# foriequal0/homework-18-graphics-raytracer

Measured on AMD Instinct MI355X. Metric: Mrays/s (primary+secondary) at 1920x1080, depth 8, higher is better.
Workload: dtype f32

## Files before the change

### homework-18-graphics-raytracer_amd/csrc/rt_pwf.hip

```cpp
#include "rt_pwf_kernel.h"

namespace rt {

static size_t pwf_dynamic_lds(uint32_t node_cap, uint32_t ring_cap) {
    const bool packed = pa_ready_packed(node_cap, ring_cap);
    return (size_t)(PA_READY_WORDS((node_cap + 63u) / 64u, packed) + 2u * PA_READY_WORDS(ring_cap / 64u, packed)) * sizeof(uint32_t);
}

int pwf_workgroups_per_cu(uint32_t node_cap, uint32_t ring_cap, bool bfs_walk) {
    int n = 0;
    const size_t lds = pwf_dynamic_lds(node_cap, ring_cap);
    const bool packed = pa_ready_packed(node_cap, ring_cap);
    const hipError_t e = bfs_walk ? (packed ? hipOccupancyMaxActiveBlocksPerMultiprocessor(&n, pwf_kernel<true, true>, (int)PA_THREADS, lds)
                                            : hipOccupancyMaxActiveBlocksPerMultiprocessor(&n, pwf_kernel<false, true>, (int)PA_THREADS, lds))
                                  : (packed ? hipOccupancyMaxActiveBlocksPerMultiprocessor(&n, pwf_kernel<true, false>, (int)PA_THREADS, lds)
                                            : hipOccupancyMaxActiveBlocksPerMultiprocessor(&n, pwf_kernel<false, false>, (int)PA_THREADS, lds));
    if (e != hipSuccess || n < 1) n = 1;
    return n;
}

__global__ void pwf_init_kernel(uint32_t *global, KernelFrame *frame, const KernelFrame fr) {
    if (threadIdx.x < PW_G_BLOCK_WORDS) global[threadIdx.x] = 0u;
    if (threadIdx.x == 0u) *frame = fr;
}

size_t pwf_arena_bytes(uint32_t node_cap, uint32_t ring_cap, uint32_t max_depth) {
    return ((size_t)node_cap * 4u + (size_t)ring_cap * (3u + PA_SHADE_U4)) * sizeof(uint4) + (size_t)(node_cap / 64u) * 2u * sizeof(uint32_t) +
           (((size_t)node_cap + 15u) & ~(size_t)15u) + (size_t)pwf_fold_list_regions(max_depth) * node_cap * sizeof(uint32_t) + 256u;
}

#ifdef PA_STATS
static uint32_t *g_pw_last_global = nullptr;
extern "C" int rt_diag_read_pwf(uint32_t *out32) {
    if (!g_pw_last_global) return -1;
    return hipMemcpy(out32, g_pw_last_global, 32 * sizeof(uint32_t), hipMemcpyDeviceToHost) == hipSuccess ? 0 : -1;
}
extern "C" int rt_diag_read_pwf_phases(unsigned long long *out32, int reset) {
    if (hipMemcpyFromSymbol(out32, HIP_SYMBOL(pa_phase_stats), 32 * sizeof(unsigned long long)) != hipSuccess) return -1;
    if (reset) {
        unsigned long long zero[32] = {0};
        if (hipMemcpyToSymbol(HIP_SYMBOL(pa_phase_stats), zero, sizeof zero) != hipSuccess) return -1;
    }
    return 0;
}
#endif

hipError_t launch_pwf(const KernelScene &sc, KernelFrame fr, float *out, const PwParams &pp, uint32_t workgroups, hipStream_t stream,
                      bool init, bool first_band, bool last_band) {
    const uint32_t total = fr.cols * fr.rows;
    fr.n_chunks = (total + 63u) / 64u;
    if (total == 0u) return hipSuccess;
#ifdef PA_STATS
    g_pw_last_global = pp.global;
#endif
    if (init) hipLaunchKernelGGL(pwf_init_kernel, dim3(1), dim3(64), 0, stream, pp.global, const_cast<KernelFrame *>(pp.frame), fr);
    if (first_band) record_main_kernel_event(0, stream);
    const size_t lds = pwf_dynamic_lds(pp.node_cap, pp.ring_cap);
    const bool packed = pa_ready_packed(pp.node_cap, pp.ring_cap);
    if (frame_is_rays(fr)) launch_pwf_rays(sc, pp, out, workgroups, lds, stream, packed, sc.bfs_walk != 0u && pp.bfs_scratch != nullptr);
    else launch_pwf_kernel<false>(sc, pp, out, workgroups, lds, stream, packed, sc.bfs_walk != 0u && pp.bfs_scratch != nullptr);
    if (last_band) record_main_kernel_event(1, stream);
    return hipGetLastError();
}

}

#ifdef RT_DIAG_STAGES
RT_DIAG_STAGE_READER(rt_diag_read_stages_pwf)
#endif
#ifdef RT_DIAG_NEED
RT_DIAG_NEED_READER(rt_diag_read_need_pwf)
#endif
#ifdef RT_DIAG_BFS
RT_DIAG_BFS_READER(rt_diag_read_bfs)
#endif
```

### homework-18-graphics-raytracer_amd/csrc/rt_pwf_kernel.h

```cpp
#ifndef RT_PWF_KERNEL_H
#define RT_PWF_KERNEL_H

#include <hip/hip_runtime.h>
#include <stdint.h>

#include "../../include/rt_amd.h"
#include "rt_device_scene.h"
#include "rt_shade.h"
#include "rt_kernels.h"
#include "rt_cast.h"
#include "rt_pwf_common.h"

namespace rt {

#ifndef PA_WAVES
#define PA_WAVES 8u
#endif
#define PA_THREADS (PA_WAVES * 64u)
#ifndef PA_MIN_WAVES
#define PA_MIN_WAVES 6
#endif
#ifndef PA_SHADE_PAGES
#define PA_SHADE_PAGES 4u
#endif
#ifndef PA_MIN_PARTIAL
#define PA_MIN_PARTIAL 1u
#endif
#ifndef PA_CHAIN_PARTIAL_MIN
#define PA_CHAIN_PARTIAL_MIN 1u
#endif
#ifndef PA_PRIO_CHAIN
#define PA_PRIO_CHAIN 1
#define PA_PRIO_TILE 1
#endif
#ifndef PA_SLEEP
#define PA_SLEEP 16
#endif
#define PA_SHADE_U4 5u
#ifndef PA_LDS_PAGES
#define PA_LDS_PAGES 2u
#endif
#ifndef PA_LQ
#define PA_LQ 3u
#endif
#define PA_LQ_SHIFT 4u
#ifndef PA_LDS_F_PAGES
#define PA_LDS_F_PAGES 2u
#endif
#ifndef PA_LDS_N_PAGES
#define PA_LDS_N_PAGES 2u
#endif
#ifndef PA_DRAIN_ROOM
#define PA_DRAIN_ROOM 64u
#endif
#define PA_IN_LDS 8u
#define PA_SPIN_LIMIT (1u << 22)

enum : uint32_t { PA_T_NONE = 0u, PA_T_NODE = 1u, PA_T_REFR = 2u, PA_T_TILE = 3u, PA_T_SHADE = 4u };

struct PaShared {
    PaQueue n, f, s;
    PaQueue l[PA_LQ];
    uint32_t l_released[PA_LQ];
    uint32_t ready_l[PA_LQ][PA_LDS_PAGES];
    PaQueue lf;
    uint32_t lf_released;
    uint32_t ready_lf[PA_LDS_F_PAGES];
    PaQueue ln;
    uint32_t ln_released;
    uint32_t ready_ln[PA_LDS_N_PAGES];
    uint32_t root_alloc;
    uint32_t tiles_exhausted;
    uint32_t tile_list_count;
    uint32_t static_next;
    uint32_t idle;
    uint32_t gen;
    uint32_t done;
    uint32_t abort;
    uint32_t fold_count[64];
};

template <class P>
__device__ __forceinline__ void pa_store_shade(P *t, uint32_t id, uint32_t prim, uint32_t word, V3 spos, V3 adj_n, V3 in_dir, V3 sdiffuse, V3 sum) {
    t[PA_F(0u)] = make_uint4(id, prim, word, 0u);
    t[PA_F(1u)] = make_uint4(pfu(spos.x), pfu(spos.y), pfu(spos.z), pfu(sum.x));
    t[PA_F(2u)] = make_uint4(pfu(adj_n.x), pfu(adj_n.y), pfu(adj_n.z), pfu(sum.y));
    t[PA_F(3u)] = make_uint4(pfu(in_dir.x), pfu(in_dir.y), pfu(in_dir.z), pfu(sum.z));
    t[PA_F(4u)] = make_uint4(pfu(sdiffuse.x), pfu(sdiffuse.y), pfu(sdiffuse.z), 0u);
}

template <class P>
__device__ __forceinline__ void pa_store_node(P *t, V3 o, V3 d, uint32_t word, float contribution, uint32_t id) {
    t[PA_F(0u)] = make_uint4(pfu(o.x), pfu(o.y), pfu(o.z), pfu(d.x));
    t[PA_F(1u)] = make_uint4(pfu(d.y), pfu(d.z), word, pfu(contribution));
    if (id != 0xffffffffu) t[PA_F(2u)] = make_uint4(id, 0u, 0u, 0u);
}

__device__ __forceinline__ uint32_t pa_top_node(uint32_t *root_alloc, const uint32_t *n_alloc, uint32_t node_cap, bool want, bool *overflow) {
    const unsigned long long mask = __builtin_amdgcn_ballot_w64(want);
    *overflow = false;
    if (mask == 0ull) return 0u;
    const uint32_t n = (uint32_t)__builtin_popcountll(mask);
    const int leader = (int)__builtin_ctzll(mask);
    uint32_t base = 0u;
    if ((int)(threadIdx.x & 63u) == leader) base = atomicAdd(root_alloc, n);
    base = (uint32_t)__builtin_amdgcn_readlane((int)base, leader);
    if (base + n + lds_load(n_alloc) > node_cap) { *overflow = want; return 0u; }
    return node_cap - 1u - (base + __builtin_amdgcn_mbcnt_hi((uint32_t)(mask >> 32), __builtin_amdgcn_mbcnt_lo((uint32_t)mask, 0u)));
}

template <class P>
__device__ __forceinline__ void pa_store_refr(P *t, V3 o, V3 d, uint32_t word, uint32_t parent, uint32_t obj, float contribution, float travel, uint32_t retry) {
    t[PA_F(0u)] = make_uint4(pfu(o.x), pfu(o.y), pfu(o.z), pfu(d.x));
    t[PA_F(1u)] = make_uint4(pfu(d.y), pfu(d.z), word, parent);
    t[PA_F(2u)] = make_uint4(obj, pfu(contribution), pfu(travel), retry);
}

__device__ __forceinline__ void pa_release_page(uint32_t *released, uint32_t page, uint32_t lane) {
    asm volatile("s_waitcnt lgkmcnt(0)" ::: "memory");
    if (lane == 0u) {
        while (lds_load(released) != page) __builtin_amdgcn_s_sleep(1);
        __hip_atomic_store(released, page + 1u, __ATOMIC_RELEASE, __HIP_MEMORY_SCOPE_WORKGROUP);
    }
}

#ifdef PA_STATS
__device__ unsigned long long pa_phase_stats[32];
#define PA_TICK() __builtin_readcyclecounter()
#endif

template <bool PACKED, bool BFS = false, bool RAYS = false>
__global__ __launch_bounds__(PA_THREADS, BFS ? 2 : PA_MIN_WAVES) void pwf_kernel(const KernelScene sc, const PwParams pp, float *__restrict__ out) {
    BfsLds *bfs_lds = nullptr;
    BfsScratch bfs_ws = {nullptr, nullptr, nullptr, 0u, 0u};
    if constexpr (BFS) {
        __shared__ BfsLds bfs_lds_all[PA_WAVES];
        bfs_lds = &bfs_lds_all[threadIdx.x >> 6];
        uint2 *const mine = reinterpret_cast<uint2 *>(pp.bfs_scratch) + ((size_t)blockIdx.x * PA_WAVES + (threadIdx.x >> 6)) * (2u * (size_t)pp.bfs_items_cap + pp.bfs_jobs_cap);
        bfs_ws.items_a = mine;
        bfs_ws.items_b = mine + pp.bfs_items_cap;
        bfs_ws.jobs = mine + 2u * (size_t)pp.bfs_items_cap;
        bfs_ws.items_cap = pp.bfs_items_cap;
        bfs_ws.jobs_cap = pp.bfs_jobs_cap;
    }
    extern __shared__ uint32_t pa_ready[];
    __shared__ PaShared S;
    __shared__ uint4 lds_shade[PA_LQ * PA_LDS_PAGES * PA_SHADE_U4 * 64u];
    __shared__ uint4 lds_refr[PA_LDS_F_PAGES * 3u * 64u];
    __shared__ uint4 lds_node[PA_LDS_N_PAGES * 3u * 64u];
    const auto &fr = uniform_ref(pp.frame);
    const uint32_t lane = threadIdx.x & 63u;
    const uint32_t total_slots = fr.cols * fr.rows;
    const uint32_t n_tiles = fr.n_chunks;
    const float THRESHOLD = 0.001f;

    unsigned char *arena = pp.arena + (size_t)blockIdx.x * pp.arena_stride;
    uint4 *node_in = reinterpret_cast<uint4 *>(arena);
    uint4 *nodes = node_in + (size_t)pp.node_cap * 2u;
    uint4 *shade_q = nodes + (size_t)pp.node_cap * 2u;
    uint4 *refr_q = shade_q + (size_t)pp.ring_cap * PA_SHADE_U4;
    uint32_t *tile_list = reinterpret_cast<uint32_t *>(refr_q + (size_t)pp.ring_cap * 3u);
    const uint32_t ring_mask = pp.ring_cap - 1u;
    const uint32_t tile_cap = pp.node_cap / 64u;
    unsigned char *root_mark = reinterpret_cast<unsigned char *>(((uintptr_t)(tile_list + (size_t)tile_cap * 2u) + 15u) & ~(uintptr_t)15u);
    uint32_t *fold_list = reinterpret_cast<uint32_t *>(root_mark + (((size_t)pp.node_cap + 15u) & ~(size_t)15u));
    auto fold_slot = [&](uint32_t level, uint32_t i) -> uint32_t * {
        uint32_t *region = fold_list + (size_t)((level - 1u) >> 1) * pp.node_cap;
        return region + (((level - 1u) & 1u) != 0u ? pp.node_cap - 1u - i : i);
    };
    const uint32_t node_pages = (pp.node_cap + 63u) / 64u, ring_pages = pp.ring_cap / 64u;
    uint32_t *ready_n = pa_ready, *ready_s = pa_ready + PA_READY_WORDS(node_pages, PACKED), *ready_f = ready_s + PA_READY_WORDS(ring_pages, PACKED);
    const uint32_t ring_page_mask = ring_pages - 1u;

    for (uint32_t i = threadIdx.x; i < PA_READY_WORDS(node_pages, PACKED) + 2u * PA_READY_WORDS(ring_pages, PACKED); i += PA_THREADS) pa_ready[i] = 0u;
    if (threadIdx.x < 64u) S.fold_count[threadIdx.x] = 0u;
    if (threadIdx.x == 0u) {
        S.n.alloc = S.n.taken = 0u;
        S.f.alloc = S.f.taken = 0u;
        S.s.alloc = S.s.taken = 0u;
        for (uint32_t q = 0; q < PA_LQ; ++q) {
            S.l[q].alloc = S.l[q].taken = 0u;
            S.l_released[q] = 0u;
            for (uint32_t k = 0; k < PA_LDS_PAGES; ++k) S.ready_l[q][k] = 0u;
        }
        S.lf.alloc = S.lf.taken = 0u;
        S.lf_released = 0u;
        for (uint32_t k = 0; k < PA_LDS_F_PAGES; ++k) S.ready_lf[k] = 0u;
        S.ln.alloc = S.ln.taken = 0u;
        S.ln_released = 0u;
        for (uint32_t k = 0; k < PA_LDS_N_PAGES; ++k) S.ready_ln[k] = 0u;
        S.root_alloc = 0u;
        S.tiles_exhausted = 0u;
        S.tile_list_count = 0u;
        S.static_next = 0u;
        S.idle = 0u;
        S.gen = 0u;
        S.done = 0u;
        S.abort = 0u;
    }
    __syncthreads();
    uint32_t casts = 0u;
    auto queue_shade = [&](bool want, uint32_t id, uint32_t prim, uint32_t word, uint32_t light_i, V3 spos, V3 adj_n, V3 in_dir, V3 sdiffuse, V3 sum) {
        const uint32_t mine = light_i < PA_LQ - 1u ? light_i : PA_LQ - 1u;
#pragma unroll
        for (uint32_t q = 0; q < PA_LQ; ++q) {
            const bool w = want && mine == q;
            if (__builtin_amdgcn_ballot_w64(w) == 0ull) continue;
            bool fits;
            const uint32_t k = pa_try_append_some(&S.l[q], &S.l_released[q], PA_LDS_PAGES * 64u, w, &fits);
            if (fits) pa_store_shade(lds_shade + q * (PA_LDS_PAGES * PA_SHADE_U4 * 64u) + pa_entry(k & (PA_LDS_PAGES * 64u - 1u), PA_SHADE_U4), id, prim, word, spos, adj_n, in_dir, sdiffuse, sum);
            pa_publish(S.ready_l[q], PA_LDS_PAGES - 1u, fits, k, &S.gen);
            want = want && !fits;
        }
#ifdef PA_STATS
        for (uint32_t q = 0; q < 3u; ++q) {
            const unsigned long long m = __builtin_amdgcn_ballot_w64(want && (mine < 2u ? mine : 2u) == q);
            if (m != 0ull && lane == (uint32_t)__builtin_ctzll(m)) atomicAdd(pp.global + 28 + q, (uint32_t)__builtin_popcountll(m));
        }
#endif
        const uint32_t k = lds_append(&S.s.alloc, want);
        if (want) pa_store_shade(shade_q + pa_entry(k & ring_mask, PA_SHADE_U4), id, prim, word, spos, adj_n, in_dir, sdiffuse, sum);
        pa_publish<PACKED>(ready_s, ring_page_mask, want, k, &S.gen);
    };
#ifdef PA_STATS
    const unsigned long long st_t0 = __builtin_amdgcn_s_memrealtime();
    uint32_t st_hist[5] = {0u, 0u, 0u, 0u, 0u};
    uint32_t st_shadow[3] = {0u, 0u, 0u};
    unsigned long long ph[26];
    for (int k = 0; k < 26; ++k) ph[k] = 0ull;
#endif

    for (;;) {
        if (lds_load(&S.done) != 0u || lds_load(&S.abort) != 0u) break;

#ifdef PA_STATS
        const unsigned long long ph_t0 = PA_TICK();
#endif
        uint32_t type = PA_T_NONE, start = 0u, count = 0u;
        if (lane == 0u) {
            const uint32_t gen = lds_load(&S.gen);
            auto look = [&]() -> uint32_t {
                const uint32_t a0 = lds_load(&S.ln.alloc), a1 = lds_load(&S.n.alloc), a2 = lds_load(&S.lf.alloc), a3 = lds_load(&S.f.alloc);
                const uint32_t t0 = lds_load(&S.ln.taken), t1 = lds_load(&S.n.taken), t2 = lds_load(&S.lf.taken), t3 = lds_load(&S.f.taken);
                uint32_t al[PA_LQ], tl[PA_LQ];
                for (uint32_t q = 0; q < PA_LQ; ++q) { al[q] = lds_load(&S.l[q].alloc); tl[q] = lds_load(&S.l[q].taken); }
                const uint32_t as = lds_load(&S.s.alloc), ts = lds_load(&S.s.taken);
                uint32_t m = (a0 > t0 * 64u ? 1u : 0u) | (a1 > t1 * 64u ? 2u : 0u) | (a2 > t2 * 64u ? 4u : 0u) | (a3 > t3 * 64u ? 8u : 0u);
                for (uint32_t q = 0; q < PA_LQ; ++q) m |= al[q] > tl[q] * 64u ? 16u << q : 0u;
                m |= as > ts * 64u ? 16u << PA_LQ : 0u;
                return m;
            };
            uint32_t have = look();
            auto claim_chain = [&](uint32_t min_partial) {
                if ((have & 1u) != 0u) {
                    count = pa_claim(&S.ln, S.ready_ln, PA_LDS_N_PAGES - 1u, min_partial, &start);
                    if (count != 0u) { type = PA_T_NODE | PA_IN_LDS; return; }
                }
                if ((have & 2u) != 0u) {
                    count = pa_claim<PACKED>(&S.n, ready_n, 0xffffffffu, min_partial, &start);
                    if (count != 0u) { type = PA_T_NODE; return; }
                }
                if ((have & 4u) != 0u) {
                    count = pa_claim(&S.lf, S.ready_lf, PA_LDS_F_PAGES - 1u, min_partial, &start);
                    if (count != 0u) { type = PA_T_REFR | PA_IN_LDS; return; }
                }
                if ((have & 8u) != 0u) {
                    count = pa_claim<PACKED>(&S.f, ready_f, ring_page_mask, min_partial, &start);
                    if (count != 0u) type = PA_T_REFR;
                }
            };
            auto claim_shade = [&](uint32_t min_partial) {
                for (uint32_t q = 0; q < PA_LQ; ++q) {
                    if ((have & (16u << q)) == 0u) continue;
                    count = pa_claim(&S.l[q], S.ready_l[q], PA_LDS_PAGES - 1u, min_partial, &start);
                    if (count != 0u) { type = PA_T_SHADE | PA_IN_LDS | (q << PA_LQ_SHIFT); return; }
                }
                if ((have & (16u << PA_LQ)) == 0u) return;
                count = pa_claim<PACKED>(&S.s, ready_s, ring_page_mask, min_partial, &start);
                if (count != 0u) type = PA_T_SHADE;
            };
            claim_chain(0u);
            if (PA_DRAIN_ROOM != 0u && type == PA_T_NONE && lds_load(&S.tiles_exhausted) == 0u) {
                for (uint32_t q = 0; q < PA_LQ; ++q) {
                    if (lds_load(&S.l[q].alloc) - (lds_load(&S.l_released[q]) << 6) + PA_DRAIN_ROOM > PA_LDS_PAGES * 64u) {
                        count = pa_claim(&S.l[q], S.ready_l[q], PA_LDS_PAGES - 1u, 0u, &start);
                        if (count != 0u) { type = PA_T_SHADE | PA_IN_LDS | (q << PA_LQ_SHIFT); break; }
                    }
                }
            }
            if (PA_CHAIN_PARTIAL_MIN != 0u && type == PA_T_NONE) claim_chain(PA_CHAIN_PARTIAL_MIN);
            bool tried_tile = false;
            for (int pass = 0; pass < 2 && type == PA_T_NONE; ++pass) {
                if (!tried_tile && lds_load(&S.tiles_exhausted) == 0u) {
                    uint32_t shade_pages = (lds_load(&S.s.alloc) >> 6) - lds_load(&S.s.taken);
                    for (uint32_t q = 0; q < PA_LQ; ++q) shade_pages += (lds_load(&S.l[q].alloc) >> 6) - lds_load(&S.l[q].taken);
                    if (pass == 1 || (int32_t)shade_pages < (int32_t)PA_SHADE_PAGES) {
                        tried_tile = true;
                        const uint32_t used = lds_load(&S.n.alloc) + lds_load(&S.root_alloc);
                        const uint32_t room = pp.node_cap > used ? pp.node_cap - used : 0u;
                        if (room < 64u * pp.tile_reserve || lds_load(&S.tile_list_count) >= tile_cap) {
                            S.tiles_exhausted = 1u;
                        } else {
                            const uint32_t share = n_tiles / gridDim.x;
                            const uint32_t own = share / 2u > (share < 8u ? share : 8u) ? share / 2u : (share < 8u ? share : 8u);
                            uint32_t k;
                            const uint32_t mine = own != 0u && lds_load(&S.static_next) < own ? atomicAdd(&S.static_next, 1u) : own;
                            if (mine < own) k = blockIdx.x + gridDim.x * mine;
                            else k = gridDim.x * own + atomicAdd(pp.global + PW_G_TILE, 1u);
                            if (k >= n_tiles) {
                                S.tiles_exhausted = 1u;
                            } else {
                                start = pp.tile_order != nullptr ? pp.tile_order[k] : (uint32_t)(((unsigned long long)k * pp.tile_stride) % n_tiles);
                                count = total_slots - start * 64u < 64u ? total_slots - start * 64u : 64u;
                                type = PA_T_TILE;
                            }
                        }
                    }
                }
                if (type == PA_T_NONE && pass == 0) claim_shade(0u);
            }
            for (int last = 0; last < 2 && type == PA_T_NONE; ++last) {
                const uint32_t min_partial = last ? 1u : PA_MIN_PARTIAL;
                have = look();
                claim_chain(min_partial);
                if (type != PA_T_NONE) break;
                claim_shade(min_partial);
                if (type != PA_T_NONE) break;
                if (last) {
                    if (lds_load(&S.idle) == PA_WAVES - 1u) S.done = 1u;
                    break;
                }
                if (atomicAdd(&S.idle, 1u) + 1u == PA_WAVES) {
                    atomicSub(&S.idle, 1u);
                    continue;
                }
                uint32_t spins = 0u;
                while (lds_load(&S.gen) == gen && lds_load(&S.done) == 0u && lds_load(&S.abort) == 0u) {
                    __builtin_amdgcn_s_sleep(PA_SLEEP);
                    if (++spins > PA_SPIN_LIMIT) {
                        S.abort = 1u;
                        atomicExch(pp.global + PW_G_OVERFLOW, 1u);
                    }
                }
                atomicSub(&S.idle, 1u);
                break;
            }
        }
        type = (uint32_t)__builtin_amdgcn_readfirstlane((int)type);
        start = (uint32_t)__builtin_amdgcn_readfirstlane((int)start);
        count = (uint32_t)__builtin_amdgcn_readfirstlane((int)count);
        const bool in_lds = (type & PA_IN_LDS) != 0u;
        const uint32_t lq = (type >> PA_LQ_SHIFT) & 3u;
        type &= 7u;
        const bool one_light = type == PA_T_SHADE && in_lds && (lq < PA_LQ - 1u || sc.n_lights <= PA_LQ);
#ifdef PA_STATS
        const unsigned long long ph_t1 = PA_TICK();
        if (type == PA_T_NONE) ph[24] += ph_t1 - ph_t0;
        const uint32_t ph_k = type == PA_T_NODE ? 0u : (type == PA_T_REFR ? 1u : (type == PA_T_TILE ? 2u : 3u));
#endif
        if (type == PA_T_NONE) continue;
        __builtin_amdgcn_fence(__ATOMIC_ACQUIRE, "workgroup");
        if (type == PA_T_SHADE) __builtin_amdgcn_s_setprio(0);
        else if (type == PA_T_TILE) __builtin_amdgcn_s_setprio(PA_PRIO_TILE);
        else __builtin_amdgcn_s_setprio(PA_PRIO_CHAIN);
#ifdef PA_STATS
        st_hist[count <= 8u ? 0 : (count <= 16u ? 1 : (count <= 32u ? 2 : (count < 64u ? 3 : 4)))] += 1u;
#endif

        const bool active = lane < count;
        Ray req;
        req.o = v3(0.0f, 0.0f, 0.0f);
        req.d = v3(0.0f, 0.0f, 1.0f);
        req.mode = FACE_FRONT;
        req.excl = 0u;
        bool do_cast = active;
        uint32_t id = 0u;
        uint32_t depth = 0u;
        float contribution = 1.0f;
        uint32_t obj = 0u;
        float travel = 0.0f;
        int32_t retry = -1;
        uint32_t prim = 0u, light_i = 0u, sflags = 0u;
        V3 spos = v3(0.0f, 0.0f, 0.0f), adj_n = v3(0.0f, 0.0f, 1.0f), in_dir = v3(0.0f, 0.0f, 1.0f), sdiffuse = spos, sum = spos;
        DirLight dl;
        dl.direction = dl.color = v3(0.0f, 0.0f, 0.0f);
        bool from_tile = false;

        if (type == PA_T_TILE) {
            const uint32_t tile = start;
            uint32_t base = 0u, entry = 0u;
            if (lane == 0u) {
                base = atomicAdd(&S.root_alloc, count);
                entry = atomicAdd(&S.tile_list_count, 1u);
            }
            base = (uint32_t)__builtin_amdgcn_readfirstlane((int)base);
            entry = (uint32_t)__builtin_amdgcn_readfirstlane((int)entry);
            if (base + count + lds_load(&S.n.alloc) > pp.node_cap || entry >= tile_cap) {
                if (lane == 0u) { S.abort = 1u; atomicExch(pp.global + PW_G_OVERFLOW, 1u); }
                break;
            }
            const uint32_t first_id = pp.node_cap - base - count;
            if (lane == 0u) { tile_list[entry * 2u] = tile; tile_list[entry * 2u + 1u] = first_id; }
            id = first_id + lane;
            depth = (uint32_t)(fr.max_depth > 0 ? fr.max_depth : 0);
            if constexpr (RAYS) {
                contribution = frame_root_contribution(fr);
                if (active) req = ray_from_abi(frame_rays(fr) + (tile * 64u + lane), sc.n_triangles, sc.n_spheres);
                do_cast = active && !(contribution < THRESHOLD);
            } else if (active) {
                uint32_t row, col;
                pw_slot_to_pixel(fr, tile * 64u + lane, &row, &col);
                const uint32_t x = fr.x0 + col, y = fr.y0 + row * fr.y_step;
                const float clip_y = (fr.half_height - (float)y) / fr.height_f;
                const float clip_x = ((float)x - fr.half_width) / fr.height_f;
                const V3 cx = v3(fr.cam_x[0], fr.cam_x[1], fr.cam_x[2]);
                const V3 cy = v3(fr.cam_y[0], fr.cam_y[1], fr.cam_y[2]);
                const V3 ct = v3(fr.cam_toward[0], fr.cam_toward[1], fr.cam_toward[2]);
                req.o = v3(fr.cam_origin[0], fr.cam_origin[1], fr.cam_origin[2]);
                req.d = normalize(clip_x * cx + clip_y * cy + ct);
            }
            type = PA_T_NODE;
            from_tile = true;
        } else if (type == PA_T_NODE) {
            uint4 a, b;
            a = b = make_uint4(0u, 0u, 0u, 0u);
            if (in_lds) {
                if (active) {
                    const uint4 *t = lds_node + pa_entry((start + lane) & (PA_LDS_N_PAGES * 64u - 1u), 3u);
                    a = t[PA_F(0u)], b = t[PA_F(1u)];
                    id = t[PA_F(2u)].x;
                }
                pa_release_page(&S.ln_released, start >> 6, lane);
            } else {
                id = start + lane;
                if (active) a = node_in[pa_entry(id, 2u)], b = node_in[pa_entry(id, 2u) + PA_F(1u)];
            }
            if (active) {
                req.o = v3(puf(a.x), puf(a.y), puf(a.z));
                req.d = v3(puf(a.w), puf(b.x), puf(b.y));
                req.mode = (b.z >> PW_MODE_SHIFT) & 3u;
                depth = (b.z >> PW_DEPTH_SHIFT) & 63u;
                req.excl = b.z & PW_EXCL_MASK;
                contribution = puf(b.w);
            }
        } else if (type == PA_T_REFR) {
            uint4 a, b, c;
            a = b = c = make_uint4(0u, 0u, 0u, 0u);
            if (in_lds) {
                if (active) {
                    const uint4 *t = lds_refr + pa_entry((start + lane) & (PA_LDS_F_PAGES * 64u - 1u), 3u);
                    a = t[PA_F(0u)], b = t[PA_F(1u)], c = t[PA_F(2u)];
                }
                pa_release_page(&S.lf_released, start >> 6, lane);
            } else if (active) {
                const uint4 *t = refr_q + pa_entry((start + lane) & ring_mask, 3u);
                a = t[PA_F(0u)], b = t[PA_F(1u)], c = t[PA_F(2u)];
            }
            if (active) {
                req.o = v3(puf(a.x), puf(a.y), puf(a.z));
                req.d = v3(puf(a.w), puf(b.x), puf(b.y));
                req.mode = (b.z >> PW_MODE_SHIFT) & 3u;
                depth = (b.z >> PW_DEPTH_SHIFT) & 63u;
                req.excl = b.z & PW_EXCL_MASK;
                id = b.w;
                obj = c.x;
                contribution = puf(c.y);
                travel = puf(c.z);
                retry = (int32_t)c.w;
            }
        } else {
            uint4 a, b, c, d, e;
            a = b = c = d = e = make_uint4(0u, 0u, 0u, 0u);
            if (in_lds) {
                if (active) {
                    const uint4 *t = lds_shade + lq * (PA_LDS_PAGES * PA_SHADE_U4 * 64u) + pa_entry((start + lane) & (PA_LDS_PAGES * 64u - 1u), PA_SHADE_U4);
                    a = t[PA_F(0u)], b = t[PA_F(1u)], c = t[PA_F(2u)], d = t[PA_F(3u)], e = t[PA_F(4u)];
                }
                pa_release_page(&S.l_released[lq], start >> 6, lane);
            } else if (active) {
                const uint4 *t = shade_q + pa_entry((start + lane) & ring_mask, PA_SHADE_U4);
                a = t[PA_F(0u)], b = t[PA_F(1u)], c = t[PA_F(2u)], d = t[PA_F(3u)], e = t[PA_F(4u)];
            }
            if (active) {
                id = a.x; prim = a.y; obj = a.z & 0xffffu; light_i = (a.z >> 16) & 0x3fffu; sflags = a.z >> 30;
                spos = v3(puf(b.x), puf(b.y), puf(b.z)); sum.x = puf(b.w);
                adj_n = v3(puf(c.x), puf(c.y), puf(c.z)); sum.y = puf(c.w);
                in_dir = v3(puf(d.x), puf(d.y), puf(d.z)); sum.z = puf(d.w);
                sdiffuse = v3(puf(e.x), puf(e.y), puf(e.z));
                if (one_light) do_cast = approximate_into_directional(uniform_ref(sc.lights + lq), spos, &dl);
                else do_cast = next_shadow_ray(sc, &light_i, spos, adj_n, &dl);
                req.o = spos;
                req.d = -dl.direction;
                req.mode = FACE_BACK;
                req.excl = pack_excl(prim, FACE_BACK);
            }
        }

#ifdef PA_STATS
        const unsigned long long ph_t2 = PA_TICK();
#endif
        CastResult cr;
        cr.prim = -1;
        cr.t = 0.0f;
        cr.bf = 0u;
        cr.a0 = cr.a1 = cr.a2 = 0.0f;
        if constexpr (BFS) {
            cr = cast_bfs(sc, req, do_cast, bfs_lds, bfs_ws);
            if (do_cast) casts += 1u;
        } else if (do_cast) {
            cr = cast_asm(sc, req);
            casts += 1u;
        }
#ifdef PA_STATS
        const unsigned long long ph_t3 = PA_TICK();
#endif

        if (type == PA_T_NODE) {
            V3 acc = v3(0.0f, 0.0f, 0.0f);
            float rc = 0.0f, fc = 0.0f;
            uint32_t rec_cr = PW_FINAL, rec_cf = PW_NO_CHILD;
            bool want_shade = false, want_refl = false, want_refr = false;
            HitGeom nh;
            nh.pos = nh.normal = v3(0.0f, 0.0f, 0.0f);
            nh.u = nh.v = 0.0f;
            nh.prim = nh.bf = nh.obj = 0u;
            V3 inside_d = v3(0.0f, 0.0f, 0.0f);
            if (active && cr.prim >= 0) {
                nh = finish_hit(sc, req, cr, false);
                const rt_material &rm = sc.materials[nh.obj];
                const float shade_contribution = (1.0f - rm.shiness) * (1.0f - rm.transparency);
                want_shade = contribution * shade_contribution >= THRESHOLD;
                if (depth > 0u) {
                    acc = v3(0.0f, 0.0f, 0.0f) * shade_contribution;
                    rc = rm.shiness * (1.0f - rm.transparency);
                    fc = rm.transparency;
                    rec_cr = PW_NO_CHILD;
                    want_refl = contribution * rc >= THRESHOLD;
                    if (contribution * fc > THRESHOLD) {
                        V3 refract_in;
                        if (refract_dir(nh.normal, req.d, rm.refraction_index, &refract_in)) {
                            inside_d = normalize(refract_in);
                            want_refr = true;
                        }
                    }
                }
            }
            bool refl_in_lds, overflow;
            const uint32_t q_refl = pa_try_append(&S.ln, &S.ln_released, PA_LDS_N_PAGES * 64u, want_refl, &refl_in_lds);
            const uint32_t k_refl = refl_in_lds ? pa_top_node(&S.root_alloc, &S.n.alloc, pp.node_cap, want_refl, &overflow)
                                                : lds_append(&S.n.alloc, want_refl);
            if (!refl_in_lds) overflow = want_refl && k_refl + lds_load(&S.root_alloc) >= pp.node_cap;
            if (want_refl && !overflow) rec_cr = k_refl;
            const bool below = active && cr.prim >= 0 && depth > 0u && (want_refl || want_refr);
            const bool bare = active && cr.prim >= 0 && depth > 0u && !below;
            if (active) {
                if (below) nodes[pa_entry(id, 2u) + PA_F(1u)] = make_uint4(pfu(fc), 0u, rec_cr, rec_cf);
                if (from_tile) root_mark[id] = (unsigned char)(below ? 0u : 0xffu);
            }
            if (want_refl && !overflow) {
                const V3 d = reflect_dir(nh.normal, req.d);
                const uint32_t word = pack_excl(nh.prim, nh.bf ? FACE_FRONT : FACE_BACK) | (req.mode << PW_MODE_SHIFT) | ((depth - 1u) << PW_DEPTH_SHIFT);
                if (refl_in_lds) pa_store_node(lds_node + pa_entry(q_refl & (PA_LDS_N_PAGES * 64u - 1u), 3u), nh.pos, d, word, contribution * rc, k_refl);
                else pa_store_node(node_in + pa_entry(k_refl, 2u), nh.pos, d, word, contribution * rc, 0xffffffffu);
            }
            bool refr_in_lds;
            uint32_t k_refr = pa_try_append(&S.lf, &S.lf_released, PA_LDS_F_PAGES * 64u, want_refr, &refr_in_lds);
            if (!refr_in_lds) k_refr = lds_append(&S.f.alloc, want_refr);
            if (want_refr) {
                const uint32_t word = pack_excl(nh.prim, FACE_FRONT) | (FACE_BACK << PW_MODE_SHIFT) | ((depth - 1u) << PW_DEPTH_SHIFT);
                if (refr_in_lds) pa_store_refr(lds_refr + pa_entry(k_refr & (PA_LDS_F_PAGES * 64u - 1u), 3u), nh.pos, inside_d, word, id, nh.obj, contribution * fc, 0.0f, 0xffffffffu);
                else pa_store_refr(refr_q + pa_entry(k_refr & ring_mask, 3u), nh.pos, inside_d, word, id, nh.obj, contribution * fc, 0.0f, 0xffffffffu);
            }
            const bool any_overflow = __builtin_amdgcn_ballot_w64(overflow) != 0ull;
            if (refl_in_lds) pa_publish(S.ready_ln, PA_LDS_N_PAGES - 1u, want_refl && !any_overflow, q_refl, &S.gen);
            else pa_publish<PACKED>(ready_n, 0xffffffffu, want_refl && !any_overflow, k_refl, &S.gen);
            if (refr_in_lds) pa_publish(S.ready_lf, PA_LDS_F_PAGES - 1u, want_refr, k_refr, &S.gen);
            else pa_publish<PACKED>(ready_f, ring_page_mask, want_refr, k_refr, &S.gen);
            if (any_overflow && lane == 0u) { S.abort = 1u; atomicExch(pp.global + PW_G_OVERFLOW, 1u); }
            if (!from_tile) {
                unsigned long long todo = __builtin_amdgcn_ballot_w64(below);
                while (todo != 0ull) {
                    const int first = (int)__builtin_ctzll(todo);
                    const uint32_t l = (uint32_t)__builtin_amdgcn_readlane((int)depth, first);
                    const bool mine = below && depth == l;
                    const unsigned long long m = __builtin_amdgcn_ballot_w64(mine);
                    uint32_t at = 0u;
                    if ((int)lane == first) at = atomicAdd(&S.fold_count[l & 63u], (uint32_t)__builtin_popcountll(m));
                    at = (uint32_t)__builtin_amdgcn_readlane((int)at, first) + __builtin_amdgcn_mbcnt_hi((uint32_t)(m >> 32), __builtin_amdgcn_mbcnt_lo((uint32_t)m, 0u));
                    if (mine) {
                        if (at < pp.node_cap) *fold_slot(l, at) = id;
                        else { S.abort = 1u; atomicExch(pp.global + PW_G_OVERFLOW, 1u); }
                    }
                    todo &= ~m;
                }
            }
            if (want_shade) {
                const rt_material &rm = sc.materials[nh.obj];
                const Mat m = material_approx(rm, nh.u, nh.v);
                adj_n = adjust_normal(m.normal, nh.normal);
                sdiffuse = m.diffuse;
                light_i = 0u;
            }
            want_shade = next_shadow_ray_in_step(sc, 0u, want_shade, &light_i, nh.pos, adj_n);
            if (active && !want_shade) {
                if (bare) { const V3 black = v3(0.0f, 0.0f, 0.0f); acc = (acc + black * rc) + black * fc; }
                nodes[pa_entry(id, 2u)] = make_uint4(pfu(acc.x), pfu(acc.y), pfu(acc.z), pfu(rc));
            }
            queue_shade(want_shade, id, nh.prim, nh.obj | (light_i << 16) | (depth > 0u ? (bare ? 0x40000000u : 0u) : 0x80000000u), light_i, nh.pos, adj_n, req.d,
                        sdiffuse, v3(0.0f, 0.0f, 0.0f));
        } else if (type == PA_T_REFR) {
            bool requeue = false, escape = false;
            V3 esc_o = v3(0.0f, 0.0f, 0.0f), esc_d = esc_o;
            uint32_t esc_excl = 0u;
            float decay = 0.0f;
            if (active && cr.prim >= 0) {
                const HitGeom ih = finish_hit(sc, req, cr, false);
                if (retry < 0) {
                    travel = distance(ih.pos, req.o);
                    retry = 0;
                } else {
                    travel += distance(req.o, ih.pos);
                    retry += 1;
                }
                const rt_material &rm = sc.materials[obj];
                V3 out_dir;
                const bool have_out = refract_dir(ih.normal, req.d, 1.0f / rm.refraction_index, &out_dir);
                if (!have_out && travel <= 100.0f && retry < 10) {
                    const V3 d = reflect_dir(ih.normal, req.d);
                    req.o = ih.pos;
                    req.d = d;
                    req.excl = pack_excl(ih.prim, ih.bf ? FACE_FRONT : FACE_BACK);
                    requeue = true;
                } else if (have_out) {
                    escape = true;
                    esc_o = ih.pos;
                    esc_d = normalize(out_dir);
                    esc_excl = pack_excl(ih.prim, FACE_BACK);
                }
            }
            bool again_in_lds;
            uint32_t k_again = pa_try_append(&S.lf, &S.lf_released, PA_LDS_F_PAGES * 64u, requeue, &again_in_lds);
            if (!again_in_lds) k_again = lds_append(&S.f.alloc, requeue);
            if (requeue) {
                const uint32_t word = req.excl | (req.mode << PW_MODE_SHIFT) | (depth << PW_DEPTH_SHIFT);
                if (again_in_lds) pa_store_refr(lds_refr + pa_entry(k_again & (PA_LDS_F_PAGES * 64u - 1u), 3u), req.o, req.d, word, id, obj, contribution, travel, (uint32_t)retry);
                else pa_store_refr(refr_q + pa_entry(k_again & ring_mask, 3u), req.o, req.d, word, id, obj, contribution, travel, (uint32_t)retry);
            }
            bool child_in_lds, overflow;
            const uint32_t q_child = pa_try_append(&S.ln, &S.ln_released, PA_LDS_N_PAGES * 64u, escape, &child_in_lds);
            const uint32_t k_child = child_in_lds ? pa_top_node(&S.root_alloc, &S.n.alloc, pp.node_cap, escape, &overflow) : lds_append(&S.n.alloc, escape);
            if (!child_in_lds) overflow = escape && k_child + lds_load(&S.root_alloc) >= pp.node_cap;
            if (escape && !overflow) {
                const uint32_t word = esc_excl | (FACE_FRONT << PW_MODE_SHIFT) | (depth << PW_DEPTH_SHIFT);
                if (child_in_lds) pa_store_node(lds_node + pa_entry(q_child & (PA_LDS_N_PAGES * 64u - 1u), 3u), esc_o, esc_d, word, contribution, k_child);
                else pa_store_node(node_in + pa_entry(k_child, 2u), esc_o, esc_d, word, contribution, 0xffffffffu);
                reinterpret_cast<uint32_t *>(nodes + pa_entry(id, 2u) + PA_F(1u))[3] = k_child;
            }
            const bool any_overflow = __builtin_amdgcn_ballot_w64(overflow) != 0ull;
            if (again_in_lds) pa_publish(S.ready_lf, PA_LDS_F_PAGES - 1u, requeue, k_again, &S.gen);
            else pa_publish<PACKED>(ready_f, ring_page_mask, requeue, k_again, &S.gen);
            if (child_in_lds) pa_publish(S.ready_ln, PA_LDS_N_PAGES - 1u, escape && !any_overflow, q_child, &S.gen);
            else pa_publish<PACKED>(ready_n, 0xffffffffu, escape && !any_overflow, k_child, &S.gen);
            if (any_overflow && lane == 0u) { S.abort = 1u; atomicExch(pp.global + PW_G_OVERFLOW, 1u); }
            if (escape && !overflow) {
                decay = rtdm::powf(sc.materials[obj].opaque_decay, travel);
                reinterpret_cast<uint32_t *>(nodes + pa_entry(id, 2u) + PA_F(1u))[1] = pfu(decay);
            }
        } else {
            bool again = false;
            if (active) {
                const rt_material &rm = sc.materials[obj];
                if (do_cast) {
                    bool lit = true;
                    if (cr.prim >= 0) {
                        auto occluded = [&](const auto &L) {
                            const bool has_origin = (L.kind != RT_LIGHT_DIRECTIONAL) || (L.has_origin != 0u);
                            if (!has_origin) return true;
                            const V3 occ = req.o + req.d * cr.t;
                            const float occlusion_distance = distance(spos, occ);
                            const float light_distance = distance(spos, v3(L.origin[0], L.origin[1], L.origin[2]));
                            return occlusion_distance < light_distance;
                        };
                        lit = one_light ? !occluded(uniform_ref(sc.lights + lq)) : !occluded(sc.lights[light_i]);
                    }
#ifdef PA_STATS
                    st_shadow[0] += 1u;
                    if (cr.prim >= 0) st_shadow[1] += 1u;
                    if (!lit) st_shadow[2] += 1u;
#endif
                    if (lit) {
                        Mat m;
                        m.normal = v3(0.0f, 0.0f, 0.0f);
                        m.diffuse = sdiffuse;
                        m.specular = v3(rm.specular_color[0], rm.specular_color[1], rm.specular_color[2]);
                        m.shiness = rm.shiness;
                        m.smoothness = rm.smoothness;
                        m.transparency = rm.transparency;
                        m.refraction_index = rm.refraction_index;
                        m.opaque_decay = rm.opaque_decay;
                        const V3 light_direction = req.d;
                        const V3 view_direction = -in_dir;
                        const V3 diffuse = get_diffuse(m, adj_n, light_direction) * dl.color;
                        const V3 specular = get_specular(m, adj_n, view_direction, light_direction) * dl.color;
                        sum = sum + diffuse * (1.0f - m.shiness) + specular * m.shiness;
                    }
                    light_i += 1u;
                    if (!one_light) again = next_shadow_ray(sc, &light_i, spos, adj_n, &dl);
                }
            }
            if (one_light) again = next_shadow_ray_in_step(sc, lq + 1u, active && do_cast, &light_i, spos, adj_n);
            if (active) {
                const rt_material &rm = sc.materials[obj];
                if (!again) {
                    V3 acc = sum;
                    float rc = 0.0f;
                    if ((sflags & 2u) == 0u) {
                        const float shade_contribution = (1.0f - rm.shiness) * (1.0f - rm.transparency);
                        acc = sum * shade_contribution;
                        rc = rm.shiness * (1.0f - rm.transparency);
                        if ((sflags & 1u) != 0u) {
                            const V3 black = v3(0.0f, 0.0f, 0.0f);
                            acc = (acc + black * rc) + black * rm.transparency;
                        }
                    }
                    nodes[pa_entry(id, 2u)] = make_uint4(pfu(acc.x), pfu(acc.y), pfu(acc.z), pfu(rc));
                }
            }
            queue_shade(again, id, prim, obj | (light_i << 16) | (sflags << 30), light_i, spos, adj_n, in_dir, sdiffuse, sum);
        }
#ifdef PA_STATS
        {
            const unsigned long long ph_t4 = PA_TICK();
            ph[0 + ph_k] += ph_t1 - ph_t0;
            ph[4 + ph_k] += ph_t2 - ph_t1;
            ph[8 + ph_k] += ph_t3 - ph_t2;
            ph[12 + ph_k] += ph_t4 - ph_t3;
            ph[16 + ph_k] += 1ull;
            ph[20 + ph_k] += count;
        }
#endif
    }

#ifdef PA_STATS
    const unsigned long long st_t1 = __builtin_amdgcn_s_memrealtime();
#endif
    __syncthreads();
#ifdef PA_STATS
    const unsigned long long st_t2 = __builtin_amdgcn_s_memrealtime();
#endif
    const bool aborted = S.abort != 0u;
    const uint32_t n_nodes = S.n.alloc < pp.node_cap ? S.n.alloc : pp.node_cap;
    const uint32_t max_depth = (uint32_t)(fr.max_depth > 0 ? fr.max_depth : 0);
    const uint32_t n_top = S.root_alloc < pp.node_cap - n_nodes ? S.root_alloc : pp.node_cap - n_nodes;
    const uint32_t top_first = pp.node_cap - n_top;
    if (!aborted) {
        auto fold_value = [&](uint32_t id, const uint4 a, const uint4 b) {
            const float rc = puf(a.w), fc = puf(b.x), decay = puf(b.y);
            V3 reflection = v3(0.0f, 0.0f, 0.0f), refraction = v3(0.0f, 0.0f, 0.0f);
            uint4 cr = make_uint4(0u, 0u, 0u, 0u), cf = cr;
            if (b.z != PW_NO_CHILD) cr = nodes[pa_entry(b.z, 2u)];
            if (b.w != PW_NO_CHILD) cf = nodes[pa_entry(b.w, 2u)];
            if (b.z != PW_NO_CHILD) reflection = v3(puf(cr.x), puf(cr.y), puf(cr.z));
            if (b.w != PW_NO_CHILD) refraction = v3(puf(cf.x), puf(cf.y), puf(cf.z)) * decay;
            const V3 value = (v3(puf(a.x), puf(a.y), puf(a.z)) + reflection * rc) + refraction * fc;
            float *rec = reinterpret_cast<float *>(nodes + pa_entry(id, 2u));
            rec[0] = value.x;
            rec[1] = value.y;
            rec[2] = value.z;
        };
        auto fold_node = [&](uint32_t id) { fold_value(id, nodes[pa_entry(id, 2u)], nodes[pa_entry(id, 2u) + PA_F(1u)]); };
        auto fold_listed = [&](uint32_t level) -> uint32_t { const uint32_t c = S.fold_count[level]; return c < pp.node_cap ? c : pp.node_cap; };
        auto first_id = [&](uint32_t level) -> uint32_t {
            return level < max_depth && threadIdx.x < fold_listed(level) ? *fold_slot(level, threadIdx.x) : PW_NO_CHILD;
        };
#ifdef PA_STATS
        const unsigned long long st_f0 = __builtin_amdgcn_s_memrealtime();
#endif
        uint32_t id0 = first_id(1u), id1 = first_id(2u);
        uint4 a0 = make_uint4(0u, 0u, 0u, 0u), b0 = a0;
        if (id0 != PW_NO_CHILD) a0 = nodes[pa_entry(id0, 2u)], b0 = nodes[pa_entry(id0, 2u) + PA_F(1u)];
        for (uint32_t left = 1u; left < max_depth; ++left) {
            const uint32_t n = fold_listed(left);
            const uint32_t id2 = first_id(left + 2u);
            uint4 a1 = make_uint4(0u, 0u, 0u, 0u), b1 = a1;
            if (id1 != PW_NO_CHILD) a1 = nodes[pa_entry(id1, 2u)], b1 = nodes[pa_entry(id1, 2u) + PA_F(1u)];
            if (id0 != PW_NO_CHILD) fold_value(id0, a0, b0);
            for (uint32_t i = threadIdx.x + PA_THREADS; i < n; i += PA_THREADS) fold_node(*fold_slot(left, i));
            __syncthreads();
            id0 = id1, a0 = a1, b0 = b1, id1 = id2;
        }
#ifdef PA_STATS
        const unsigned long long st_f1 = __builtin_amdgcn_s_memrealtime();
#endif
        const uint32_t n_started = S.tile_list_count;
        for (uint32_t e0 = threadIdx.x >> 6; e0 < n_started; e0 += PA_WAVES * 4u) {
            uint32_t id[4], slot[4], tile_of[4];
            uint4 ra[4], rb[4];
            bool live[4];
#pragma unroll
            for (uint32_t j = 0; j < 4u; ++j) {
                const uint32_t e = e0 + j * PA_WAVES;
                live[j] = false;
                id[j] = slot[j] = 0u;
                tile_of[j] = 0xffffffffu;
                if (e < n_started) {
                    const uint32_t tile = tile_list[e * 2u], base = tile_list[e * 2u + 1u];
                    tile_of[j] = tile;
                    const uint32_t first_slot = tile * 64u;
                    const uint32_t nv = total_slots - first_slot < 64u ? total_slots - first_slot : 64u;
                    live[j] = lane < nv;
                    id[j] = base + lane;
                    slot[j] = first_slot + lane;
                }
                if (live[j]) {
                    ra[j] = nodes[pa_entry(id[j], 2u)];
                    rb[j] = make_uint4(0u, 0u, PW_FINAL, PW_NO_CHILD);
                    if (root_mark[id[j]] != 0xffu) rb[j] = nodes[pa_entry(id[j], 2u) + PA_F(1u)];
                }
            }
            if (pp.tile_cost != nullptr) {
#pragma unroll
                for (uint32_t j = 0; j < 4u; ++j) {
                    const unsigned long long deep = __builtin_amdgcn_ballot_w64(live[j] && rb[j].z != PW_FINAL);
                    if (lane == 0u && tile_of[j] != 0xffffffffu) pp.tile_cost[tile_of[j]] = (uint32_t)__builtin_popcountll(deep);
                }
            }
            uint4 cr4[4], cf4[4];
#pragma unroll
            for (uint32_t j = 0; j < 4u; ++j) {
                cr4[j] = cf4[j] = make_uint4(0u, 0u, 0u, 0u);
                if (live[j] && rb[j].z != PW_FINAL) {
                    if (rb[j].z != PW_NO_CHILD) cr4[j] = nodes[pa_entry(rb[j].z, 2u)];
                    if (rb[j].w != PW_NO_CHILD) cf4[j] = nodes[pa_entry(rb[j].w, 2u)];
                }
            }
#pragma unroll
            for (uint32_t j = 0; j < 4u; ++j) {
                if (!live[j]) continue;
                const uint4 a = ra[j], b = rb[j];
                V3 value = v3(puf(a.x), puf(a.y), puf(a.z));
                if (b.z != PW_FINAL) {
                    const float rc = puf(a.w), fc = puf(b.x), decay = puf(b.y);
                    V3 reflection = v3(0.0f, 0.0f, 0.0f), refraction = v3(0.0f, 0.0f, 0.0f);
                    if (b.z != PW_NO_CHILD) reflection = v3(puf(cr4[j].x), puf(cr4[j].y), puf(cr4[j].z));
                    if (b.w != PW_NO_CHILD) refraction = v3(puf(cf4[j].x), puf(cf4[j].y), puf(cf4[j].z)) * decay;
                    value = (value + reflection * rc) + refraction * fc;
                }
                uint32_t row, col;
                pw_slot_to_pixel(fr, slot[j], &row, &col);
                float *px = out + ((size_t)row * fr.cols + col) * 3u;
                if constexpr (RAYS) {
                    px[0] = value.x;
                    px[1] = value.y;
                    px[2] = value.z;
                } else {
                    px[0] = 0.0f + value.x;
                    px[1] = 0.0f + value.y;
                    px[2] = 0.0f + value.z;
                }
            }
        }
        if (threadIdx.x == 0u && n_started != 0u) atomicAdd(pp.global + PW_G_TILES_DONE, n_started);
#ifdef PA_STATS
        __syncthreads();
        if (threadIdx.x == 0u) {
            atomicAdd(&pa_phase_stats[26], st_f0 - st_t2);
            atomicAdd(&pa_phase_stats[27], st_f1 - st_f0);
            atomicAdd(&pa_phase_stats[28], __builtin_amdgcn_s_memrealtime() - st_f1);
            atomicAdd(&pa_phase_stats[29], 1ull);
        }
#endif
    }
#ifdef PA_STATS
    __syncthreads();
    {
        const unsigned long long st_t3 = __builtin_amdgcn_s_memrealtime();
        if (lane == 0u) { atomicAdd(pp.global + 8, (uint32_t)(st_t1 - st_t0)); atomicMax(pp.global + 9, (uint32_t)(st_t1 - st_t0)); }
        if (lane == 0u) for (int k = 0; k < 5; ++k) atomicAdd(pp.global + 20 + k, st_hist[k]);
        for (int k = 0; k < 3; ++k) {
            uint32_t v = st_shadow[k];
            for (int off = 32; off > 0; off >>= 1) v += __shfl_down(v, off, 64);
            if (lane == 0u && v != 0u) atomicAdd(pp.global + (k == 0 ? 18 : (k == 1 ? 19 : 31)), v);
        }
        if (lane == 0u) {
            ph[25] = st_t3 - st_t2;
            for (int k = 0; k < 26; ++k) atomicAdd(&pa_phase_stats[k], ph[k]);
        }
        if (threadIdx.x == 0u) {
            atomicAdd(pp.global + 10, (uint32_t)(st_t2 - st_t0)); atomicMax(pp.global + 11, (uint32_t)(st_t2 - st_t0));
            atomicAdd(pp.global + 12, (uint32_t)(st_t3 - st_t2)); atomicMax(pp.global + 13, (uint32_t)(st_t3 - st_t2));
            atomicAdd(pp.global + 14, 1u); atomicAdd(pp.global + 15, S.n.alloc);
            atomicAdd(pp.global + 25, S.s.alloc); atomicAdd(pp.global + 26, S.f.alloc); atomicAdd(pp.global + 27, S.root_alloc);
            atomicMin(pp.global + 16, (uint32_t)(st_t3 - st_t0)); atomicMax(pp.global + 17, (uint32_t)(st_t3 - st_t0));
        }
    }
#endif
    if (threadIdx.x == 0u) S.gen = 0u;
    __syncthreads();
    for (int off = 32; off > 0; off >>= 1) casts += __shfl_down(casts, off, 64);
    if (lane == 0u && casts != 0u) atomicAdd(&S.gen, casts);

    __syncthreads();
    if (threadIdx.x == 0u) {
        if (S.gen != 0u) atomicAdd(reinterpret_cast<unsigned long long *>(pp.global + PW_G_CASTS), (unsigned long long)S.gen);
        __threadfence();
        if (atomicAdd(pp.global + PW_G_GROUPS_DONE, 1u) + 1u == gridDim.x) {
            __threadfence();
            uint32_t overflow = __hip_atomic_load(pp.global + PW_G_OVERFLOW, __ATOMIC_RELAXED, __HIP_MEMORY_SCOPE_AGENT);
            const uint32_t tiles_done = __hip_atomic_load(pp.global + PW_G_TILES_DONE, __ATOMIC_RELAXED, __HIP_MEMORY_SCOPE_AGENT);
            if (overflow == 0u && tiles_done != n_tiles) {
                overflow = 1u;
                atomicExch(pp.global + PW_G_OVERFLOW, 1u);
            }
            if (overflow == 0u && pp.ray_count != nullptr)
                atomicAdd(pp.ray_count,
                          __hip_atomic_load(reinterpret_cast<unsigned long long *>(pp.global + PW_G_CASTS), __ATOMIC_RELAXED, __HIP_MEMORY_SCOPE_AGENT));
            for (uint32_t k = 0; k < PW_G_BLOCK_WORDS; ++k) pp.global_next[k] = 0u;
        }
    }
}

template <bool RAYS>
static void launch_pwf_kernel(const KernelScene &sc, const PwParams &pp, float *out, uint32_t workgroups, size_t lds, hipStream_t stream, bool packed,
                              bool bfs) {
    if (bfs) {
        if (packed) hipLaunchKernelGGL((pwf_kernel<true, true, RAYS>), dim3(workgroups), dim3(PA_THREADS), lds, stream, sc, pp, out);
        else hipLaunchKernelGGL((pwf_kernel<false, true, RAYS>), dim3(workgroups), dim3(PA_THREADS), lds, stream, sc, pp, out);
    } else if (packed) hipLaunchKernelGGL((pwf_kernel<true, false, RAYS>), dim3(workgroups), dim3(PA_THREADS), lds, stream, sc, pp, out);
    else hipLaunchKernelGGL((pwf_kernel<false, false, RAYS>), dim3(workgroups), dim3(PA_THREADS), lds, stream, sc, pp, out);
}

}

#endif
```

Baseline: 18890.

## Split shade queue entries into slim queue words plus per-node global shade records

Shade-queue entries shrink from five uint4 to one, holding only a packed id/light/flags word and the running sum. The per-hit geometry (position, normal, incoming direction, diffuse, prim, obj) is written once per node into a new global shade_rec array indexed by node id. This cuts the traffic of requeueing the same hit once per light and frees LDS, so the LDS shade pages rise from 2 to 8. The trade-off is that every shade dequeue, including ones served from LDS, now does four global loads. Node ids are also masked to 16 bits, which assumes the node capacity fits in that range.

```diff
diff --git a/homework-18-graphics-raytracer_amd/csrc/rt_pwf.hip b/homework-18-graphics-raytracer_amd/csrc/rt_pwf.hip
--- a/homework-18-graphics-raytracer_amd/csrc/rt_pwf.hip
+++ b/homework-18-graphics-raytracer_amd/csrc/rt_pwf.hip
@@ -25,7 +25,7 @@
 }
 
 size_t pwf_arena_bytes(uint32_t node_cap, uint32_t ring_cap, uint32_t max_depth) {
-    return ((size_t)node_cap * 4u + (size_t)ring_cap * (3u + PA_SHADE_U4)) * sizeof(uint4) + (size_t)(node_cap / 64u) * 2u * sizeof(uint32_t) +
+    return ((size_t)node_cap * (4u + PA_SHADE_REC_U4) + (size_t)ring_cap * (3u + PA_SHADE_U4)) * sizeof(uint4) + (size_t)(node_cap / 64u) * 2u * sizeof(uint32_t) +
            (((size_t)node_cap + 15u) & ~(size_t)15u) + (size_t)pwf_fold_list_regions(max_depth) * node_cap * sizeof(uint32_t) + 256u;
 }
 
diff --git a/homework-18-graphics-raytracer_amd/csrc/rt_pwf_kernel.h b/homework-18-graphics-raytracer_amd/csrc/rt_pwf_kernel.h
--- a/homework-18-graphics-raytracer_amd/csrc/rt_pwf_kernel.h
+++ b/homework-18-graphics-raytracer_amd/csrc/rt_pwf_kernel.h
@@ -36,9 +36,10 @@
 #ifndef PA_SLEEP
 #define PA_SLEEP 16
 #endif
-#define PA_SHADE_U4 5u
+#define PA_SHADE_U4 1u
+#define PA_SHADE_REC_U4 4u
 #ifndef PA_LDS_PAGES
-#define PA_LDS_PAGES 2u
+#define PA_LDS_PAGES 8u
 #endif
 #ifndef PA_LQ
 #define PA_LQ 3u
@@ -80,13 +81,22 @@
     uint32_t fold_count[64];
 };
 
+#define PA_SHADE_LIGHT_SHIFT 16u
+#define PA_SHADE_FLAGS_SHIFT 30u
+__device__ __forceinline__ uint32_t pa_shade_word(uint32_t id, uint32_t light_i, uint32_t sflags) {
+    return id | (light_i << PA_SHADE_LIGHT_SHIFT) | (sflags << PA_SHADE_FLAGS_SHIFT);
+}
+
 template <class P>
-__device__ __forceinline__ void pa_store_shade(P *t, uint32_t id, uint32_t prim, uint32_t word, V3 spos, V3 adj_n, V3 in_dir, V3 sdiffuse, V3 sum) {
-    t[PA_F(0u)] = make_uint4(id, prim, word, 0u);
-    t[PA_F(1u)] = make_uint4(pfu(spos.x), pfu(spos.y), pfu(spos.z), pfu(sum.x));
-    t[PA_F(2u)] = make_uint4(pfu(adj_n.x), pfu(adj_n.y), pfu(adj_n.z), pfu(sum.y));
-    t[PA_F(3u)] = make_uint4(pfu(in_dir.x), pfu(in_dir.y), pfu(in_dir.z), pfu(sum.z));
-    t[PA_F(4u)] = make_uint4(pfu(sdiffuse.x), pfu(sdiffuse.y), pfu(sdiffuse.z), 0u);
+__device__ __forceinline__ void pa_store_shade(P *t, uint32_t word, V3 sum) {
+    t[0] = make_uint4(word, pfu(sum.x), pfu(sum.y), pfu(sum.z));
+}
+
+__device__ __forceinline__ void pa_store_shade_rec(uint4 *t, uint32_t prim, uint32_t obj, V3 spos, V3 adj_n, V3 in_dir, V3 sdiffuse) {
+    t[PA_F(0u)] = make_uint4(pfu(spos.x), pfu(spos.y), pfu(spos.z), prim);
+    t[PA_F(1u)] = make_uint4(pfu(adj_n.x), pfu(adj_n.y), pfu(adj_n.z), obj);
+    t[PA_F(2u)] = make_uint4(pfu(in_dir.x), pfu(in_dir.y), pfu(in_dir.z), 0u);
+    t[PA_F(3u)] = make_uint4(pfu(sdiffuse.x), pfu(sdiffuse.y), pfu(sdiffuse.z), 0u);
 }
 
 template <class P>
@@ -157,7 +167,8 @@
     unsigned char *arena = pp.arena + (size_t)blockIdx.x * pp.arena_stride;
     uint4 *node_in = reinterpret_cast<uint4 *>(arena);
     uint4 *nodes = node_in + (size_t)pp.node_cap * 2u;
-    uint4 *shade_q = nodes + (size_t)pp.node_cap * 2u;
+    uint4 *shade_rec = nodes + (size_t)pp.node_cap * 2u;
+    uint4 *shade_q = shade_rec + (size_t)pp.node_cap * PA_SHADE_REC_U4;
     uint4 *refr_q = shade_q + (size_t)pp.ring_cap * PA_SHADE_U4;
     uint32_t *tile_list = reinterpret_cast<uint32_t *>(refr_q + (size_t)pp.ring_cap * 3u);
     const uint32_t ring_mask = pp.ring_cap - 1u;
@@ -200,7 +211,7 @@
     }
     __syncthreads();
     uint32_t casts = 0u;
-    auto queue_shade = [&](bool want, uint32_t id, uint32_t prim, uint32_t word, uint32_t light_i, V3 spos, V3 adj_n, V3 in_dir, V3 sdiffuse, V3 sum) {
+    auto queue_shade = [&](bool want, uint32_t word, uint32_t light_i, V3 sum) {
         const uint32_t mine = light_i < PA_LQ - 1u ? light_i : PA_LQ - 1u;
 #pragma unroll
         for (uint32_t q = 0; q < PA_LQ; ++q) {
@@ -208,7 +219,7 @@
             if (__builtin_amdgcn_ballot_w64(w) == 0ull) continue;
             bool fits;
             const uint32_t k = pa_try_append_some(&S.l[q], &S.l_released[q], PA_LDS_PAGES * 64u, w, &fits);
-            if (fits) pa_store_shade(lds_shade + q * (PA_LDS_PAGES * PA_SHADE_U4 * 64u) + pa_entry(k & (PA_LDS_PAGES * 64u - 1u), PA_SHADE_U4), id, prim, word, spos, adj_n, in_dir, sdiffuse, sum);
+            if (fits) pa_store_shade(lds_shade + q * (PA_LDS_PAGES * PA_SHADE_U4 * 64u) + pa_entry(k & (PA_LDS_PAGES * 64u - 1u), PA_SHADE_U4), word, sum);
             pa_publish(S.ready_l[q], PA_LDS_PAGES - 1u, fits, k, &S.gen);
             want = want && !fits;
         }
@@ -219,7 +230,7 @@
         }
 #endif
         const uint32_t k = lds_append(&S.s.alloc, want);
-        if (want) pa_store_shade(shade_q + pa_entry(k & ring_mask, PA_SHADE_U4), id, prim, word, spos, adj_n, in_dir, sdiffuse, sum);
+        if (want) pa_store_shade(shade_q + pa_entry(k & ring_mask, PA_SHADE_U4), word, sum);
         pa_publish<PACKED>(ready_s, ring_page_mask, want, k, &S.gen);
     };
 #ifdef PA_STATS
@@ -469,23 +480,21 @@
                 retry = (int32_t)c.w;
             }
         } else {
-            uint4 a, b, c, d, e;
-            a = b = c = d = e = make_uint4(0u, 0u, 0u, 0u);
+            uint4 a = make_uint4(0u, 0u, 0u, 0u);
             if (in_lds) {
-                if (active) {
-                    const uint4 *t = lds_shade + lq * (PA_LDS_PAGES * PA_SHADE_U4 * 64u) + pa_entry((start + lane) & (PA_LDS_PAGES * 64u - 1u), PA_SHADE_U4);
-                    a = t[PA_F(0u)], b = t[PA_F(1u)], c = t[PA_F(2u)], d = t[PA_F(3u)], e = t[PA_F(4u)];
-                }
+                if (active) a = lds_shade[lq * (PA_LDS_PAGES * PA_SHADE_U4 * 64u) + pa_entry((start + lane) & (PA_LDS_PAGES * 64u - 1u), PA_SHADE_U4)];
                 pa_release_page(&S.l_released[lq], start >> 6, lane);
             } else if (active) {
-                const uint4 *t = shade_q + pa_entry((start + lane) & ring_mask, PA_SHADE_U4);
-                a = t[PA_F(0u)], b = t[PA_F(1u)], c = t[PA_F(2u)], d = t[PA_F(3u)], e = t[PA_F(4u)];
+                a = shade_q[pa_entry((start + lane) & ring_mask, PA_SHADE_U4)];
             }
             if (active) {
-                id = a.x; prim = a.y; obj = a.z & 0xffffu; light_i = (a.z >> 16) & 0x3fffu; sflags = a.z >> 30;
-                spos = v3(puf(b.x), puf(b.y), puf(b.z)); sum.x = puf(b.w);
-                adj_n = v3(puf(c.x), puf(c.y), puf(c.z)); sum.y = puf(c.w);
-                in_dir = v3(puf(d.x), puf(d.y), puf(d.z)); sum.z = puf(d.w);
+                id = a.x & 0xffffu; light_i = (a.x >> PA_SHADE_LIGHT_SHIFT) & 0x3fffu; sflags = a.x >> PA_SHADE_FLAGS_SHIFT;
+                sum = v3(puf(a.y), puf(a.z), puf(a.w));
+                const uint4 *r = shade_rec + pa_entry(id, PA_SHADE_REC_U4);
+                const uint4 b = r[PA_F(0u)], c = r[PA_F(1u)], d = r[PA_F(2u)], e = r[PA_F(3u)];
+                spos = v3(puf(b.x), puf(b.y), puf(b.z)); prim = b.w;
+                adj_n = v3(puf(c.x), puf(c.y), puf(c.z)); obj = c.w;
+                in_dir = v3(puf(d.x), puf(d.y), puf(d.z));
                 sdiffuse = v3(puf(e.x), puf(e.y), puf(e.z));
                 if (one_light) do_cast = approximate_into_directional(uniform_ref(sc.lights + lq), spos, &dl);
                 else do_cast = next_shadow_ray(sc, &light_i, spos, adj_n, &dl);
@@ -606,8 +615,8 @@
                 if (bare) { const V3 black = v3(0.0f, 0.0f, 0.0f); acc = (acc + black * rc) + black * fc; }
                 nodes[pa_entry(id, 2u)] = make_uint4(pfu(acc.x), pfu(acc.y), pfu(acc.z), pfu(rc));
             }
-            queue_shade(want_shade, id, nh.prim, nh.obj | (light_i << 16) | (depth > 0u ? (bare ? 0x40000000u : 0u) : 0x80000000u), light_i, nh.pos, adj_n, req.d,
-                        sdiffuse, v3(0.0f, 0.0f, 0.0f));
+            if (want_shade) pa_store_shade_rec(shade_rec + pa_entry(id, PA_SHADE_REC_U4), nh.prim, nh.obj, nh.pos, adj_n, req.d, sdiffuse);
+            queue_shade(want_shade, pa_shade_word(id, light_i, depth > 0u ? (bare ? 1u : 0u) : 2u), light_i, v3(0.0f, 0.0f, 0.0f));
         } else if (type == PA_T_REFR) {
             bool requeue = false, escape = false;
             V3 esc_o = v3(0.0f, 0.0f, 0.0f), esc_d = esc_o;
@@ -726,7 +735,7 @@
                     nodes[pa_entry(id, 2u)] = make_uint4(pfu(acc.x), pfu(acc.y), pfu(acc.z), pfu(rc));
                 }
             }
-            queue_shade(again, id, prim, obj | (light_i << 16) | (sflags << 30), light_i, spos, adj_n, in_dir, sdiffuse, sum);
+            queue_shade(again, pa_shade_word(id, light_i, sflags), light_i, sum);
         }
 #ifdef PA_STATS
         {
```

Result: no change. 18800 (-0.5%).
